# sunnyHelen/JPerceiver

Measured on AMD Instinct MI355X. Metric: train images/sec (full train step, synthetic 3-frame batches), higher is better.
Workload: dtype f32

## Files before the change

### jperceiver_amd/csrc/conv_pack.hip

```cpp
#include "conv_pack.h"
#include "igemm_p9.h"
#include "igemm_p9s.h"
#include "scale.h"
#include <algorithm>

namespace {

struct JpPackJob {
    const float* w;
    float* wp;
    long total, begin;
    int mode, p[6];
};
static_assert(sizeof(JpPackJob) == 64, "JpPackJob layout");
__host__ __device__ inline int jp_cdiv_d(int a, int b) { return (a + b - 1) / b; }

__device__ __forceinline__ float pack_slot_sum(const float* wc, int pl) {
    const int a = pl >> 3, b = (pl >> 2) & 1, r = (pl >> 1) & 1, sx = pl & 1;
    const int y0 = a ? (r ? 2 : 0) : (r ? 1 : 0), y1 = a ? (r ? 2 : 1) : (r ? 2 : 0);
    const int x0 = b ? (sx ? 2 : 0) : (sx ? 1 : 0), x1 = b ? (sx ? 2 : 1) : (sx ? 2 : 0);
    float v = 0.f;
    for (int dy = y0; dy <= y1; ++dy)
        for (int dx = x0; dx <= x1; ++dx) v += wc[dy * 3 + dx];
    return v;
// ... 165 lines not shown
        }
        default: {
            const int Cout = p[0], Cin = p[1], c_off = p[2];
            const int t = (int)(i % 9), co = (int)((i / 9) % Cout), c = (int)(i / (9 * (long)Cout));
            return w[((size_t)co * Cin + c_off + c) * 9 + 8 - t];
        }
    }
}

__device__ __forceinline__ int pack_hdr(int mode) { return (mode == PACK_SPLIT || mode == PACK_SPLITUPD || mode == PACK_SPLIT7) ? JP_PACK_HDR : 0; }
__device__ __forceinline__ float pack_scale_of(const JpPackJob& j) {
    if (!JP_PACK_HDR) return 1.f;
    if (j.mode == PACK_SPLIT || j.mode == PACK_SPLITUPD || j.mode == PACK_SPLIT7) return j.wp[0];
    if (j.mode == PACK_SPLITSEG) return *(j.wp - j.p[5]);
    return 1.f;
}
constexpr int PSL = 32;
__device__ __forceinline__ float* pack_scale_hdr(const JpPackJob& j, long* n) {
    const bool seg = j.mode == PACK_SPLITSEG && j.p[2] == 0;
    const bool upd = j.mode == PACK_SPLITUPD;
    const bool s7 = j.mode == PACK_SPLIT7;
    if (!JP_PACK_HDR || !(j.mode == PACK_SPLIT || seg || upd || s7)) return nullptr;
    *n = (long)j.p[0] * j.p[1] * ((seg || upd) ? 9 : (s7 ? 49 : j.p[4]));
    return seg ? j.wp - j.p[5] : j.wp;
}
__device__ __forceinline__ void pack_scale_zero(const JpPackJob& j) {
    long n;
    float* hdr = pack_scale_hdr(j, &n);
    if (hdr && threadIdx.x == 0) reinterpret_cast<unsigned*>(hdr)[2] = 0u;
}
__device__ __forceinline__ void pack_scale_reduce(const JpPackJob& j, int slice) {
    long n;
    float* hdr = pack_scale_hdr(j, &n);
    if (!hdr) return;
    const long per = (n + PSL - 1) / PSL, beg = slice * per, end = min(n, beg + per);
    unsigned m = 0;
    for (long i = beg + threadIdx.x; i < end; i += 256) m = max(m, jp_amag(__float_as_uint(j.w[i])));
#pragma unroll
    for (int o = 32; o > 0; o >>= 1) m = max(m, (unsigned)__shfl_xor((int)m, o, 64));
    if ((threadIdx.x & 63) == 0 && m) atomicMax(reinterpret_cast<unsigned*>(hdr) + 2, m);
}
__device__ __forceinline__ void pack_scale_finish(const JpPackJob& j) {
    long n;
    float* hdr = pack_scale_hdr(j, &n);
    if (!hdr || threadIdx.x) return;
    const int k = jp_scale_exp(hdr[2] * ((j.mode == PACK_SPLITSEG || j.mode == PACK_SPLITUPD) ? 4.f : 1.f));
    hdr[0] = jp_exp2i(k);
    hdr[1] = jp_exp2i(-k);
    hdr[2] = hdr[3] = 0.f;
}
__global__ __launch_bounds__(64) void pack_scale_zero_one_kernel(JpPackJob job) { pack_scale_zero(job); }
__global__ __launch_bounds__(256) void pack_scale_reduce_one_kernel(JpPackJob job) { pack_scale_reduce(job, blockIdx.x); }
__global__ __launch_bounds__(64) void pack_scale_finish_one_kernel(JpPackJob job) { pack_scale_finish(job); }
__global__ __launch_bounds__(64) void pack_scale_zero_kernel(const JpPackJob* __restrict__ jobs, int njobs) {
    const int q = blockIdx.x * 64 + threadIdx.x;
    if (q < njobs) { long n; float* hdr = pack_scale_hdr(jobs[q], &n); if (hdr) reinterpret_cast<unsigned*>(hdr)[2] = 0u; }
}
__global__ __launch_bounds__(256) void pack_scale_reduce_kernel(const JpPackJob* __restrict__ jobs, int njobs) {
    pack_scale_reduce(jobs[blockIdx.y], blockIdx.x);
}
__global__ __launch_bounds__(64) void pack_scale_finish_kernel(const JpPackJob* __restrict__ jobs, int njobs) {
    const int q = blockIdx.x * 64 + threadIdx.x;
    if (q < njobs) {
        long n;
        float* hdr = pack_scale_hdr(jobs[q], &n);
        if (hdr) {
            const int k = jp_scale_exp(hdr[2] * ((jobs[q].mode == PACK_SPLITSEG || jobs[q].mode == PACK_SPLITUPD) ? 4.f : 1.f));
            hdr[0] = jp_exp2i(k);
            hdr[1] = jp_exp2i(-k);
            hdr[2] = hdr[3] = 0.f;
        }
    }
}

__global__ __launch_bounds__(256) void pack_one_kernel(JpPackJob job) {
    const int hdr = pack_hdr(job.mode);
    const float sc = pack_scale_of(job);
    for (long i = (long)blockIdx.x * 256 + threadIdx.x; i < job.total - hdr; i += (long)gridDim.x * 256)
        job.wp[hdr + i] = pack_elem(job.mode, job.w, i, job.p, sc);
}

__global__ __launch_bounds__(256) void pack_replay_kernel(const JpPackJob* __restrict__ jobs, int njobs, long total) {
    const long groups = (total + 3) >> 2;
    for (long g4 = (long)blockIdx.x * 256 + threadIdx.x; g4 < groups; g4 += (long)gridDim.x * 256) {
        const long g = g4 << 2;
        int lo = 0, hi = njobs - 1;
        while (lo < hi) {
            const int mid = (lo + hi + 1) >> 1;
            if (jobs[mid].begin <= g) lo = mid; else hi = mid - 1;
        }
        const JpPackJob& j = jobs[lo];
        const long i = g - j.begin;
        if (i >= j.total) continue;
        if (j.mode == PACK_SPLIT || j.mode == PACK_SPLITSEG) continue;
        if (j.mode == PACK_FRAG && i + 4 <= j.total) {
            const int* p = j.p;
            const int Cout = p[0], Cin = p[1], for_dgrad = p[2], BMT = p[3], KHW = p[4];
            const int rows = for_dgrad ? Cin : Cout, red = for_dgrad ? Cout : Cin;
            const long per_tile = ((long)((red + 31) / 32) * KHW * 4 + P9_QAHEAD + 1) * 8 * BMT;
            const int mt = (int)(i / per_tile);
            long t = (i - (long)mt * per_tile) >> 2;
            const int m = mt * BMT + (int)(t % BMT);
            t /= BMT;
            const int par = (int)(t & 1); t >>= 1;
            const long step = t * 4;
            const int s0 = (int)(step & 15);
            const long tc = step >> 4;
            const int tap = (int)(tc % KHW), c0 = (int)(tc / KHW) * 32 + 2 * s0 + par;
            float4 v = make_float4(0.f, 0.f, 0.f, 0.f);
            if (m < rows) {
                const size_t cs = for_dgrad ? (size_t)Cin * KHW : (size_t)KHW;
                const float* wb = j.w + (for_dgrad ? (size_t)m * KHW : (size_t)m * Cin * KHW) + tap;
                if (c0 < red) v.x = wb[(size_t)c0 * cs];
                if (c0 + 2 < red) v.y = wb[(size_t)(c0 + 2) * cs];
                if (c0 + 4 < red) v.z = wb[(size_t)(c0 + 4) * cs];
                if (c0 + 6 < red) v.w = wb[(size_t)(c0 + 6) * cs];
            }
            *reinterpret_cast<float4*>(j.wp + i) = v;
        } else {
            const int hdr = pack_hdr(j.mode);
            const float sc = hdr ? pack_scale_of(j) : 1.f;
#pragma unroll
            for (int k = 0; k < 4; ++k)
                if (i + k >= hdr && i + k < j.total) j.wp[i + k] = pack_elem(j.mode, j.w, i + k - hdr, j.p, sc);
        }
    }
}

__device__ __forceinline__ int split_job_items(const JpPackJob& j) {
    const int* p = j.p;
    if (j.mode == PACK_SPLIT) {
        const int rows = p[2] ? p[1] : p[0], red = p[2] ? p[0] : p[1];
        return jp_cdiv_d(rows, p[3]) * (red / (16 * p[5])) * (p[3] / 64);
    }
    if (j.mode == PACK_SPLITSEG) return (p[0] / 128) * ((p[3] + 15) / 16) * 2;
    return 0;
}
__global__ __launch_bounds__(256) void pack_split_replay_kernel(const JpPackJob* __restrict__ jobs, int njobs) {
    __shared__ float tile[64 * 16 * 9 + 64];
    constexpr int MAXJ = 2048;
    __shared__ int pre[MAXJ + 1];
    const int t = threadIdx.x;
    for (int q = t; q < njobs && q < MAXJ; q += 256) pre[q + 1] = split_job_items(jobs[q]);
    if (t == 0) pre[0] = 0;
    __syncthreads();
    if (t == 0)
        for (int q = 1; q <= njobs && q <= MAXJ; ++q) pre[q] += pre[q - 1];
    __syncthreads();
    const int nj = min(njobs, MAXJ), total_items = pre[nj];
    for (int item = blockIdx.x; item < total_items; item += gridDim.x) {
        __syncthreads();
        int lo = 0, hi = nj - 1;
        while (lo < hi) {
            const int mid = (lo + hi + 1) >> 1;
            if (pre[mid] <= item) lo = mid; else hi = mid - 1;
        }
        const int jj = lo, loc = item - pre[lo];
        const JpPackJob& j = jobs[jj];
        const int* p = j.p;
        unsigned* out = reinterpret_cast<unsigned*>(j.wp) + pack_hdr(j.mode);
        if (j.mode == PACK_SPLIT) {
            const float wsc = JP_PACK_HDR ? j.wp[0] : 1.f;
            const int Cout = p[0], Cin = p[1], for_dgrad = p[2], BMT = p[3], KHW = p[4], KGS = p[5];
            const int rows = for_dgrad ? Cin : Cout, red = for_dgrad ? Cout : Cin;
            const int CS = 16 * KGS, nst = red / CS, rch = BMT / 64;
            const int rc = loc % rch, stage = (loc / rch) % nst, mt = loc / (rch * nst);
            const int m0 = mt * BMT + rc * 64, c0 = stage * CS;
            const int RUN = CS * KHW;
            if (!for_dgrad) {
                for (int e = t; e < 64 * RUN; e += 256) {
                    const int r = e / RUN, o = e - r * RUN;
                    tile[e] = (m0 + r < rows) ? j.w[((size_t)(m0 + r) * Cin + c0) * KHW + o] : 0.f;
                }
            } else {
                const int RUNd = 64 * KHW;
                for (int e = t; e < CS * RUNd; e += 256) {
                    const int c = e / RUNd, o = e - c * RUNd;
                    tile[e] = (m0 + o / KHW < rows) ? j.w[((size_t)(c0 + c) * Cin + m0) * KHW + o] : 0.f;
                }
            }
            __syncthreads();
            const long nsteps = (long)nst * KHW * KGS;
            const long per_tile = (nsteps + P9S_AHEAD) * (JP_NS * 8) * BMT;
            const int trip = KHW * KGS * 2 * 64;
            for (int e = t; e < trip; e += 256) {
                const int r = e & 63, kh = (e >> 6) & 1, u = e >> 7;
                const int tap = u / KGS, kg = u - tap * KGS;
                jp_u32x4 w0, w1, w2;
#pragma unroll
                for (int k = 0; k < 4; ++k) {
                    const int c = kg * 16 + kh * 8 + 2 * k;
                    const float a = for_dgrad ? tile[(c * 64 + r) * KHW + tap] : tile[(r * CS + c) * KHW + tap];
                    const float b = for_dgrad ? tile[((c + 1) * 64 + r) * KHW + tap] : tile[(r * CS + c + 1) * KHW + tap];
                    unsigned sq[3];
                    jp_split_ns(a, b, wsc, sq);
                    w0[k] = sq[0]; w1[k] = sq[1]; w2[k] = sq[2];
                }
                const long U = (long)stage * KHW * KGS + u;
                unsigned* q = out + (long)mt * per_tile + ((U * JP_NS) * 2 + kh) * (long)BMT * 4 + (long)(rc * 64 + r) * 4;
                *reinterpret_cast<jp_u32x4*>(q) = w0;
                *reinterpret_cast<jp_u32x4*>(q + 2L * BMT * 4) = w1;
                if (JP_NS == 3) *reinterpret_cast<jp_u32x4*>(q + 4L * BMT * 4) = w2;
            }
        } else {
            const int Cout = p[0], Cin = p[1], c_off = p[2], C = p[3], up = p[4];
            const int T = up ? 4 : 9, MT = Cout / 128, nst = (C + 15) / 16;
            const int rc = loc & 1, stage = (loc >> 1) % nst, mt = (loc >> 1) / nst;
            const int m0 = mt * 128 + rc * 64, c0 = stage * 16;
            for (int e = t; e < 64 * 144; e += 256) {
                const int r = e / 144, o = e - r * 144, c = o / 9;
                tile[e] = (c0 + c < C && m0 + r < Cout) ? j.w[((size_t)(m0 + r) * Cin + c_off + c0) * 9 + o] : 0.f;
            }
            __syncthreads();
            const long tl = (long)nst * T * (JP_NS * 1024);
            const int ncls = up ? 4 : 1, trip = ncls * T * 2 * 64;
            const float wsc = pack_scale_of(j);
            for (int e = t; e < trip; e += 256) {
                const int r = e & 63, kh = (e >> 6) & 1, ct = e >> 7, tap = ct % T, cls = ct / T;
                jp_u32x4 w0, w1, w2;
#pragma unroll
                for (int k = 0; k < 4; ++k) {
                    const int c = kh * 8 + 2 * k;
                    const float* wa = tile + (r * 16 + c) * 9;
                    const float a = up ? pack_slot_sum(wa, cls * 4 + tap) : wa[tap];
                    const float b = up ? pack_slot_sum(wa + 9, cls * 4 + tap) : wa[9 + tap];
                    unsigned sq[3];
                    jp_split_ns(a, b, wsc, sq);
                    w0[k] = sq[0]; w1[k] = sq[1]; w2[k] = sq[2];
                }
                const long U = (long)stage * T + tap;
                unsigned* q = out + (long)(cls * MT + mt) * tl + ((U * JP_NS) * 2 + kh) * 512L + (long)(rc * 64 + r) * 4;
                *reinterpret_cast<jp_u32x4*>(q) = w0;
                *reinterpret_cast<jp_u32x4*>(q + 1024) = w1;
                if (JP_NS == 3) *reinterpret_cast<jp_u32x4*>(q + 2048) = w2;
            }
        }
    }
}

thread_local JpPackJob* g_pack_rec = nullptr;
thread_local int g_pack_rec_n = 0, g_pack_rec_cap = 0;

}

void do_pack(int mode, const float* w, float* wp, long total, int p0, int p1, int p2, int p3, int p4, int p5, hipStream_t st) {
    JpPackJob j{w, wp, total, 0, mode, {p0, p1, p2, p3, p4, p5}};
    if (g_pack_rec) {
        if (g_pack_rec_n < g_pack_rec_cap) g_pack_rec[g_pack_rec_n] = j;
        ++g_pack_rec_n;
    }
    if (JP_PACK_HDR && (mode == PACK_SPLIT || mode == PACK_SPLITUPD || mode == PACK_SPLIT7 || (mode == PACK_SPLITSEG && p2 == 0))) {
        hipLaunchKernelGGL(pack_scale_zero_one_kernel, dim3(1), dim3(64), 0, st, j);
        hipLaunchKernelGGL(pack_scale_reduce_one_kernel, dim3(PSL), dim3(256), 0, st, j);
        hipLaunchKernelGGL(pack_scale_finish_one_kernel, dim3(1), dim3(64), 0, st, j);
    }
    hipLaunchKernelGGL(pack_one_kernel, dim3((int)std::min<long>((total + 255) / 256, 4096)), dim3(256), 0, st, j);
}

void pack_weights(const float* w, float* wp, int Cout, int Cin, int KHW, int Cp, int for_dgrad, hipStream_t st) {
    do_pack(PACK_TAP, w, wp, (long)KHW * (for_dgrad ? Cin : Cout) * Cp, Cout, Cin, KHW, Cp, for_dgrad, 0, st);
}

extern "C" int jp_pack_job_bytes(void) { return (int)sizeof(JpPackJob); }

extern "C" int jp_pack_record_begin(void* host_jobs, int max_jobs) {
    JP_CHECK_ARG(host_jobs && max_jobs > 0 && !g_pack_rec, "pack_record_begin: bad args or a recording is already open");
    g_pack_rec = (JpPackJob*)host_jobs;
    g_pack_rec_n = 0;
    g_pack_rec_cap = max_jobs;
    return JP_OK;
}

extern "C" int jp_pack_record_end(void) {
    g_pack_rec = nullptr;
    return g_pack_rec_n;
}

extern "C" int jp_pack_mode_is_split(int mode) { return (mode == PACK_SPLIT || mode == PACK_SPLITSEG) ? 1 : 0; }
extern "C" int jp_pack_replay(const void* jobs, int njobs, long total_elems, long generic_elems, void* stream) {
    JP_CHECK_ARG(jobs && njobs > 0 && total_elems > 0, "pack_replay: bad args");
    const long gen = (generic_elems > 0 && generic_elems < total_elems) ? generic_elems : total_elems;
    if (JP_PACK_HDR)
    {
        hipLaunchKernelGGL(pack_scale_zero_kernel, dim3((njobs + 63) / 64), dim3(64), 0, (hipStream_t)stream, (const JpPackJob*)jobs, njobs);
        hipLaunchKernelGGL(pack_scale_reduce_kernel, dim3(PSL, njobs), dim3(256), 0, (hipStream_t)stream, (const JpPackJob*)jobs, njobs);
        hipLaunchKernelGGL(pack_scale_finish_kernel, dim3((njobs + 63) / 64), dim3(64), 0, (hipStream_t)stream, (const JpPackJob*)jobs, njobs);
    }
    hipLaunchKernelGGL(pack_replay_kernel, dim3((int)std::min<long>((gen + 4095) / 4096, 16384)), dim3(256), 0,
                       (hipStream_t)stream, (const JpPackJob*)jobs, njobs, gen);
    for (int off = 0; off < njobs; off += 2048)
        hipLaunchKernelGGL(pack_split_replay_kernel, dim3(4096), dim3(256), 0, (hipStream_t)stream, (const JpPackJob*)jobs + off,
                           std::min(2048, njobs - off));
    JP_LAUNCH_CHECK();
}
```

### jperceiver_amd/csrc/pointwise.hip

```cpp
#include "jp_common.h"
#include "bilinear.h"
#include <algorithm>

namespace {

constexpr int TPB = 256;
inline int blocks_for(long n) { return (int)std::min<long>((n + TPB - 1) / TPB, 1 << 20); }

constexpr int MP_TW = 64, MP_TH = 8;

__global__ __launch_bounds__(TPB) void maxpool_fwd_kernel(const float* __restrict__ x, float* __restrict__ y,
                                                          uint8_t* __restrict__ idx, int H, int W, int OH, int OW,
                                                          int k, int s, int p) {
    extern __shared__ float tile[];
    const size_t nc = blockIdx.z;
    const float* xp = x + nc * H * W;
    const int ox0 = blockIdx.x * MP_TW, oy0 = blockIdx.y * MP_TH;
    const int pw = (MP_TW - 1) * s + k, ph = (MP_TH - 1) * s + k;
    const int ix0 = ox0 * s - p, iy0 = oy0 * s - p;
    for (int i = threadIdx.x; i < pw * ph; i += TPB) {
        const int ly = i / pw, lx = i - ly * pw;
        const int iy = iy0 + ly, ix = ix0 + lx;
        tile[i] = ((unsigned)iy < (unsigned)H && (unsigned)ix < (unsigned)W) ? xp[iy * W + ix] : -INFINITY;
    }
// ... 628 lines not shown
            mx = fmaxf(mx, jp_fmag(o));
            fs += o;
            if (++run == 32) { s += fs; fs = 0.f; run = 0; }
        }
    }
    jp_block_amax_commit(mx, amax);
    s += fs;
    s = jp_block_sum_d(s, sm);
    if (threadIdx.x == 0) {
        if (part) part[(size_t)c * gridDim.y + blockIdx.y] = (float)s;
        else atomicAdd(&dbias[c], (float)s);
    }
}
__global__ void bias_fold_kernel(const float* __restrict__ part, float* __restrict__ dbias, int C, int S) {
    const int c = blockIdx.x * blockDim.x + threadIdx.x;
    if (c >= C) return;
    float s = 0.f;
    for (int i = 0; i < S; ++i) s += part[(size_t)c * S + i];
    dbias[c] += s;
}

__global__ __launch_bounds__(TPB) void mul_bcast_c_kernel(const float* __restrict__ a, const float* __restrict__ s,
                                                          float* __restrict__ out, long total, int C, int HW) {
    for (long i = (long)blockIdx.x * TPB + threadIdx.x; i < total; i += (long)gridDim.x * TPB) {
        const int p = (int)(i % HW);
        const long n = i / ((long)C * HW);
        out[i] = a[i] * s[n * HW + p];
    }
}
__global__ __launch_bounds__(TPB) void mul_bcast_c_bwd_s_kernel(const float* __restrict__ dout,
                                                                const float* __restrict__ a, float* __restrict__ ds,
                                                                long total, int C, int HW) {
    for (long i = (long)blockIdx.x * TPB + threadIdx.x; i < total; i += (long)gridDim.x * TPB) {
        const int p = (int)(i % HW);
        const long n = i / HW;
        float g = 0.f;
        for (int c = 0; c < C; ++c) g += dout[(n * C + c) * HW + p] * a[(n * C + c) * HW + p];
        ds[i] = g;
    }
}

__global__ __launch_bounds__(TPB) void bilinear_fwd_kernel(const float* __restrict__ x, float* __restrict__ y,
                                                           long total, int H, int W, int OH, int OW, float sy,
                                                           float sx) {
    for (long o = (long)blockIdx.x * TPB + threadIdx.x; o < total; o += (long)gridDim.x * TPB) {
        const int ox = (int)(o % OW);
        const long t = o / OW;
        const int oy = (int)(t % OH);
        const long nc = t / OH;
        y[o] = bil_sample(x + nc * H * W, oy, ox, H, W, sy, sx);
    }
}

__global__ __launch_bounds__(TPB) void bilinear_bwd_kernel(const float* __restrict__ dy, float* __restrict__ dx,
                                                           long total, int H, int W, int OH, int OW, float sy,
                                                           float sx, int accumulate) {
    for (long i = (long)blockIdx.x * TPB + threadIdx.x; i < total; i += (long)gridDim.x * TPB) {
        const int ix = (int)(i % W);
        const long t = i / W;
        const int iy = (int)(t % H);
        const long nc = t / H;
        const float* dp = dy + nc * OH * OW;
        int oy_lo = max(0, (int)floorf(((float)iy - 0.5f) / sy - 0.5f) - 1);
        int oy_hi = min(OH - 1, (int)ceilf(((float)iy + 1.5f) / sy - 0.5f) + 1);
        int ox_lo = max(0, (int)floorf(((float)ix - 0.5f) / sx - 0.5f) - 1);
        int ox_hi = min(OW - 1, (int)ceilf(((float)ix + 1.5f) / sx - 0.5f) + 1);
        if (iy == 0) oy_lo = 0;
        if (ix == 0) ox_lo = 0;
        if (iy == H - 1) oy_hi = OH - 1;
        if (ix == W - 1) ox_hi = OW - 1;
        float g = 0.f;
        for (int oy = oy_lo; oy <= oy_hi; ++oy) {
            int y0, y1;
            float wy;
            bil_src(oy, sy, H, y0, y1, wy);
            float cy = 0.f;
            if (y0 == iy) cy += 1.f - wy;
            if (y1 == iy) cy += wy;
            if (cy == 0.f) continue;
            for (int ox = ox_lo; ox <= ox_hi; ++ox) {
                int x0, x1;
                float wx;
                bil_src(ox, sx, W, x0, x1, wx);
                float cx = 0.f;
                if (x0 == ix) cx += 1.f - wx;
                if (x1 == ix) cx += wx;
                if (cx != 0.f) g += cy * cx * dp[oy * OW + ox];
            }
        }
        dx[i] = accumulate ? dx[i] + g : g;
    }
}

__global__ __launch_bounds__(TPB) void area_down_kernel(const float* __restrict__ x, float* __restrict__ y,
                                                        long total, int H, int W, int OH, int OW, int f) {
    const float inv = 1.f / (float)(f * f);
    for (long o = (long)blockIdx.x * TPB + threadIdx.x; o < total; o += (long)gridDim.x * TPB) {
        const int ox = (int)(o % OW);
        const long t = o / OW;
        const int oy = (int)(t % OH);
        const long nc = t / OH;
        const float* xp = x + (nc * H + (long)oy * f) * W + (long)ox * f;
        float s = 0.f;
        for (int a = 0; a < f; ++a)
            for (int b = 0; b < f; ++b) s += xp[a * W + b];
        y[o] = s * inv;
    }
}

__global__ __launch_bounds__(TPB) void warp_perspective_kernel(const float* __restrict__ src,
                                                               const float* __restrict__ Hm, float* __restrict__ dst,
                                                               int h, int w, int OH, int OW) {
    const int b = blockIdx.y;
    const float* M = Hm + 9 * b;
    const float* sp = src + (size_t)b * h * w;
    for (int p = blockIdx.x * TPB + threadIdx.x; p < OH * OW; p += gridDim.x * TPB) {
        const int oy = p / OW, ox = p - oy * OW;
        const float gx = OW > 1 ? -1.f + 2.f * (float)ox / (float)(OW - 1) : -1.f;
        const float gy = OH > 1 ? -1.f + 2.f * (float)oy / (float)(OH - 1) : -1.f;
        const float X = M[0] * gx + M[1] * gy + M[2];
        const float Y = M[3] * gx + M[4] * gy + M[5];
        const float Z = M[6] * gx + M[7] * gy + M[8];
        const float sx = X / Z, sy = Y / Z;
        const float ix = ((sx + 1.f) * (float)w - 1.f) * 0.5f, iy = ((sy + 1.f) * (float)h - 1.f) * 0.5f;
        const float fx = floorf(ix), fy = floorf(iy);
        const int x0 = (int)fx, y0 = (int)fy;
        const float tx = ix - fx, ty = iy - fy;
        float v = 0.f;
        if (ix == ix && iy == iy && fx > -2.f && fy > -2.f && fx < (float)w + 1.f && fy < (float)h + 1.f) {
            const bool xa = x0 >= 0 && x0 < w, xb = x0 + 1 >= 0 && x0 + 1 < w;
            const bool ya = y0 >= 0 && y0 < h, yb = y0 + 1 >= 0 && y0 + 1 < h;
            if (ya && xa) v += sp[y0 * w + x0] * (1.f - tx) * (1.f - ty);
            if (ya && xb) v += sp[y0 * w + x0 + 1] * tx * (1.f - ty);
            if (yb && xa) v += sp[(y0 + 1) * w + x0] * (1.f - tx) * ty;
            if (yb && xb) v += sp[(y0 + 1) * w + x0 + 1] * tx * ty;
        }
        dst[(size_t)b * OH * OW + p] = v;
    }
}

__global__ __launch_bounds__(TPB) void softmax_c2_kernel(const float* __restrict__ x, float* __restrict__ y,
                                                         long total, int HW) {
    for (long i = (long)blockIdx.x * TPB + threadIdx.x; i < total; i += (long)gridDim.x * TPB) {
// ... 307 lines not shown
    int ch = std::max(1, 2048 / std::max(1, N * C));
    ch = std::min(ch, std::max(1, HW / 2048));
    int ck = (HW + ch - 1) / ch;
    ck = (ck + 3) & ~3;
    *chunk = ck;
    *CH = (HW + ck - 1) / ck;
}
extern "C" long jp_act_bwd_bias_ws_floats(int N, int C, int HW) {
    int CH, chunk;
    act_bias_chunks(N, C, HW, &CH, &chunk);
    return (long)C * N * CH;
}
extern "C" int jp_act_bwd_bias(const float* dy, const float* y, float* dx, float* dbias, int N, int C, int HW, int act,
                               float* amax_dx, float* bias_ws, void* stream) {
    JP_CHECK_ARG(dy && y && dx && dbias && N > 0 && C > 0 && HW > 0 && C <= 65535, "act_bwd_bias: bad args");
    JP_ST;
    int CH, chunk;
    act_bias_chunks(N, C, HW, &CH, &chunk);
    JP_CHECK_ARG((long)N * CH <= 65535, "act_bwd_bias: too many chunks");
    hipLaunchKernelGGL(act_bwd_bias_kernel, dim3(C, N * CH), dim3(TPB), 0, st, dy, y, dx, dbias, C, HW, CH, chunk, act,
                       reinterpret_cast<unsigned*>(amax_dx), bias_ws);
    if (bias_ws) hipLaunchKernelGGL(bias_fold_kernel, dim3(jp_cdiv(C, 64)), dim3(64), 0, st, bias_ws, dbias, C, N * CH);
    JP_LAUNCH_CHECK();
}

extern "C" int jp_mul_bcast_c(const float* a, const float* s, float* out, int N, int C, int HW, void* stream) {
    JP_CHECK_ARG(a && s && out && N > 0, "mul_bcast_c: bad args");
    JP_ST;
    const long total = (long)N * C * HW;
    hipLaunchKernelGGL(mul_bcast_c_kernel, dim3(blocks_for(total)), dim3(TPB), 0, st, a, s, out, total, C, HW);
    JP_LAUNCH_CHECK();
}

extern "C" int jp_mul_bcast_c_bwd_s(const float* dout, const float* a, float* ds, int N, int C, int HW,
                                    void* stream) {
    JP_CHECK_ARG(dout && a && ds && N > 0, "mul_bcast_c_bwd_s: bad args");
    JP_ST;
    const long total = (long)N * HW;
    hipLaunchKernelGGL(mul_bcast_c_bwd_s_kernel, dim3(blocks_for(total)), dim3(TPB), 0, st, dout, a, ds, total, C, HW);
    JP_LAUNCH_CHECK();
}

extern "C" int jp_bilinear_fwd(const float* x, float* y, int NC, int H, int W, int OH, int OW, void* stream) {
    JP_CHECK_ARG(x && y && NC > 0 && OH > 0 && OW > 0, "bilinear_fwd: bad args");
    JP_ST;
    const long total = (long)NC * OH * OW;
    hipLaunchKernelGGL(bilinear_fwd_kernel, dim3(blocks_for(total)), dim3(TPB), 0, st, x, y, total, H, W, OH, OW,
                       (float)H / (float)OH, (float)W / (float)OW);
    JP_LAUNCH_CHECK();
}

extern "C" int jp_bilinear_bwd(const float* dy, float* dx, int NC, int H, int W, int OH, int OW, int accumulate,
                               void* stream) {
    JP_CHECK_ARG(dy && dx && NC > 0, "bilinear_bwd: bad args");
    JP_ST;
    const long total = (long)NC * H * W;
    hipLaunchKernelGGL(bilinear_bwd_kernel, dim3(blocks_for(total)), dim3(TPB), 0, st, dy, dx, total, H, W, OH, OW,
                       (float)H / (float)OH, (float)W / (float)OW, accumulate);
    JP_LAUNCH_CHECK();
}

extern "C" int jp_area_downsample(const float* x, float* y, int NC, int H, int W, int f, void* stream) {
    JP_CHECK_ARG(x && y && NC > 0 && f >= 1 && H % f == 0 && W % f == 0, "area_downsample: bad args");
    JP_ST;
    const long total = (long)NC * (H / f) * (W / f);
    hipLaunchKernelGGL(area_down_kernel, dim3(blocks_for(total)), dim3(TPB), 0, st, x, y, total, H, W, H / f, W / f, f);
    JP_LAUNCH_CHECK();
}

extern "C" int jp_warp_perspective(const float* src, const float* Hm, float* dst, int B, int h, int w, int OH, int OW,
                                   void* stream) {
    JP_CHECK_ARG(src && Hm && dst && B > 0, "warp_perspective: bad args");
    JP_ST;
    hipLaunchKernelGGL(warp_perspective_kernel, dim3(std::min(jp_cdiv((long)OH * OW, TPB), 4096), B), dim3(TPB), 0, st,
                       src, Hm, dst, h, w, OH, OW);
    JP_LAUNCH_CHECK();
}

extern "C" int jp_softmax_c2(const float* x, float* y, int N, int HW, void* stream) {
    JP_CHECK_ARG(x && y && N > 0 && HW > 0, "softmax_c2: bad args");
    JP_ST;
    const long total = (long)N * HW;
    hipLaunchKernelGGL(softmax_c2_kernel, dim3(blocks_for(total)), dim3(TPB), 0, st, x, y, total, HW);
    JP_LAUNCH_CHECK();
}

extern "C" int jp_disp_to_depth(const float* disp, float* depth, long n, float min_depth, float max_depth,
                                void* stream) {
    JP_CHECK_ARG(disp && depth && n > 0, "disp_to_depth: bad args");
    JP_ST;
    hipLaunchKernelGGL(disp_to_depth_kernel, dim3(blocks_for(n)), dim3(TPB), 0, st, disp, depth, n, 1.f / max_depth,
                       1.f / min_depth);
    JP_LAUNCH_CHECK();
}

extern "C" int jp_fill_convex_poly(const int* pts, int npts, uint8_t* mask, int H, int W, void* stream) {
    JP_CHECK_ARG(pts && mask && npts >= 1 && npts <= POLY_MAX && H > 0 && W > 0, "fill_convex_poly: bad args");
    JP_ST;
    JP_HIP(hipMemsetAsync(mask, 0, (size_t)H * W, st));
    hipLaunchKernelGGL(fill_convex_poly_kernel, dim3(8), dim3(TPB), 0, st, pts, npts, mask, H, W);
    JP_LAUNCH_CHECK();
}

extern "C" int jp_scale_label_assemble(const float* zwarp, const float* laywarp, const uint8_t* polymask, float* out,
                                       int B, int H, int W, int mode, void* stream) {
    JP_CHECK_ARG(zwarp && out && B > 0 && (mode == 0 || polymask), "scale_label_assemble: bad args");
    JP_ST;
    const long total = (long)B * H * W;
    hipLaunchKernelGGL(scale_label_kernel, dim3(blocks_for(total)), dim3(TPB), 0, st, zwarp, laywarp, polymask, out,
                       total, (long)H * W, mode);
    JP_LAUNCH_CHECK();
// ... 2 lines not shown
```

Measured before the change: 128.5.

## Restructure weight-pack replay and separable bilinear backward with shared-memory staging

Weight packing now builds its job prefix with a parallel wave scan and runs the scale-max reduction as a flat work list with vectorized loads. Several more pack modes (tap, up-dgrad, split-update) are staged through shared-memory tiles with coalesced run fills, and launch sizes are tied to the CU count. Bilinear backward becomes separable: each block reduces the output rows into a shared horizontal buffer once, then each thread gathers along x. This cuts repeated per-pixel window scans and redundant global reads. The cost is more code and a risk of mishandling edge cases.

```diff
diff --git a/jperceiver_amd/csrc/conv_pack.hip b/jperceiver_amd/csrc/conv_pack.hip
--- a/jperceiver_amd/csrc/conv_pack.hip
+++ b/jperceiver_amd/csrc/conv_pack.hip
@@ -241,12 +241,84 @@
 __global__ __launch_bounds__(64) void pack_scale_zero_one_kernel(JpPackJob job) { pack_scale_zero(job); }
 __global__ __launch_bounds__(256) void pack_scale_reduce_one_kernel(JpPackJob job) { pack_scale_reduce(job, blockIdx.x); }
 __global__ __launch_bounds__(64) void pack_scale_finish_one_kernel(JpPackJob job) { pack_scale_finish(job); }
-__global__ __launch_bounds__(64) void pack_scale_zero_kernel(const JpPackJob* __restrict__ jobs, int njobs) {
-    const int q = blockIdx.x * 64 + threadIdx.x;
-    if (q < njobs) { long n; float* hdr = pack_scale_hdr(jobs[q], &n); if (hdr) reinterpret_cast<unsigned*>(hdr)[2] = 0u; }
+constexpr int PACK_MAXJ = 2048;
+template <class F>
+__device__ __forceinline__ int pack_item_prefix(const JpPackJob* __restrict__ jobs, int nj, int* pre, F items_of) {
+    constexpr int PER = PACK_MAXJ / 256;
+    __shared__ int wave_sum[4];
+    const int t = threadIdx.x, lane = t & 63, wv = t >> 6;
+    int cnt[PER], sum = 0;
+#pragma unroll
+    for (int k = 0; k < PER; ++k) {
+        const int q = t * PER + k;
+        cnt[k] = q < nj ? items_of(jobs[q]) : 0;
+        sum += cnt[k];
+    }
+    int inc = sum;
+#pragma unroll
+    for (int o = 1; o < 64; o <<= 1) {
+        const int v = __shfl_up(inc, o, 64);
+        if (lane >= o) inc += v;
+    }
+    if (lane == 63) wave_sum[wv] = inc;
+    __syncthreads();
+    int run = inc - sum;
+    for (int k = 0; k < wv; ++k) run += wave_sum[k];
+    if (t == 0) pre[0] = 0;
+#pragma unroll
+    for (int k = 0; k < PER; ++k) {
+        const int q = t * PER + k;
+        run += cnt[k];
+        if (q < nj) pre[q + 1] = run;
+    }
+    __syncthreads();
+    return pre[nj];
+}
+__device__ __forceinline__ int pack_item_job(const int* pre, int nj, int item) {
+    int lo = 0, hi = nj - 1;
+    while (lo < hi) {
+        const int mid = (lo + hi + 1) >> 1;
+        if (pre[mid] <= item) lo = mid; else hi = mid - 1;
+    }
+    return lo;
+}
+
+constexpr int PACK_RED_ITEM = 16384;
+__device__ __forceinline__ int scale_job_items(const JpPackJob& j) {
+    long n;
+    return pack_scale_hdr(j, &n) ? (int)((n + PACK_RED_ITEM - 1) / PACK_RED_ITEM) : 0;
 }
 __global__ __launch_bounds__(256) void pack_scale_reduce_kernel(const JpPackJob* __restrict__ jobs, int njobs) {
-    pack_scale_reduce(jobs[blockIdx.y], blockIdx.x);
+    __shared__ int pre[PACK_MAXJ + 1];
+    __shared__ unsigned wave_max[4];
+    const int t = threadIdx.x;
+    const int total_items = pack_item_prefix(jobs, njobs, pre, scale_job_items);
+    for (int item = blockIdx.x; item < total_items; item += gridDim.x) {
+        const int jj = pack_item_job(pre, njobs, item);
+        const JpPackJob& j = jobs[jj];
+        long n;
+        float* hdr = pack_scale_hdr(j, &n);
+        const long beg = (long)(item - pre[jj]) * PACK_RED_ITEM, end = min(n, beg + PACK_RED_ITEM);
+        const float* w = j.w;
+        const long a0 = min(end, beg + (long)((4 - (int)((reinterpret_cast<size_t>(w + beg) >> 2) & 3)) & 3));
+        const long nv = (end - a0) >> 2;
+        unsigned m = 0;
+        for (long i = beg + t; i < a0; i += 256) m = max(m, jp_amag(__float_as_uint(w[i])));
+        for (long i = t; i < nv; i += 256) {
+            const jp_u32x4 v = *reinterpret_cast<const jp_u32x4*>(w + a0 + 4 * i);
+            m = max(max(m, jp_amag(v[0])), max(max(jp_amag(v[1]), jp_amag(v[2])), jp_amag(v[3])));
+        }
+        for (long i = a0 + 4 * nv + t; i < end; i += 256) m = max(m, jp_amag(__float_as_uint(w[i])));
+#pragma unroll
+        for (int o = 32; o > 0; o >>= 1) m = max(m, (unsigned)__shfl_xor((int)m, o, 64));
+        if ((t & 63) == 0) wave_max[t >> 6] = m;
+        __syncthreads();
+        if (t == 0) {
+            m = max(max(wave_max[0], wave_max[1]), max(wave_max[2], wave_max[3]));
+            if (m) atomicMax(reinterpret_cast<unsigned*>(hdr) + 2, m);
+        }
+        __syncthreads();
+    }
 }
 __global__ __launch_bounds__(64) void pack_scale_finish_kernel(const JpPackJob* __restrict__ jobs, int njobs) {
     const int q = blockIdx.x * 64 + threadIdx.x;
@@ -269,53 +341,61 @@
         job.wp[hdr + i] = pack_elem(job.mode, job.w, i, job.p, sc);
 }
 
+__host__ __device__ inline bool pack_mode_staged(int mode) {
+    return mode == PACK_SPLIT || mode == PACK_SPLITSEG || mode == PACK_TAP || mode == PACK_UP_DGRAD || mode == PACK_SPLITUPD;
+}
+__device__ __forceinline__ void pack_replay_group(const JpPackJob& j, long i) {
+    if (i >= j.total) return;
+    if (pack_mode_staged(j.mode)) return;
+    if (j.mode == PACK_FRAG && i + 4 <= j.total) {
+        const int* p = j.p;
+        const int Cout = p[0], Cin = p[1], for_dgrad = p[2], BMT = p[3], KHW = p[4];
+        const int rows = for_dgrad ? Cin : Cout, red = for_dgrad ? Cout : Cin;
+        const long per_tile = ((long)((red + 31) / 32) * KHW * 4 + P9_QAHEAD + 1) * 8 * BMT;
+        const int mt = (int)(i / per_tile);
+        long t = (i - (long)mt * per_tile) >> 2;
+        const int m = mt * BMT + (int)(t % BMT);
+        t /= BMT;
+        const int par = (int)(t & 1); t >>= 1;
+        const long step = t * 4;
+        const int s0 = (int)(step & 15);
+        const long tc = step >> 4;
+        const int tap = (int)(tc % KHW), c0 = (int)(tc / KHW) * 32 + 2 * s0 + par;
+        float4 v = make_float4(0.f, 0.f, 0.f, 0.f);
+        if (m < rows) {
+            const size_t cs = for_dgrad ? (size_t)Cin * KHW : (size_t)KHW;
+            const float* wb = j.w + (for_dgrad ? (size_t)m * KHW : (size_t)m * Cin * KHW) + tap;
+            if (c0 < red) v.x = wb[(size_t)c0 * cs];
+            if (c0 + 2 < red) v.y = wb[(size_t)(c0 + 2) * cs];
+            if (c0 + 4 < red) v.z = wb[(size_t)(c0 + 4) * cs];
+            if (c0 + 6 < red) v.w = wb[(size_t)(c0 + 6) * cs];
+        }
+        *reinterpret_cast<float4*>(j.wp + i) = v;
+    } else {
+        const int hdr = pack_hdr(j.mode);
+        const float sc = hdr ? pack_scale_of(j) : 1.f;
+#pragma unroll
+        for (int k = 0; k < 4; ++k)
+            if (i + k >= hdr && i + k < j.total) j.wp[i + k] = pack_elem(j.mode, j.w, i + k - hdr, j.p, sc);
+    }
+}
+
 __global__ __launch_bounds__(256) void pack_replay_kernel(const JpPackJob* __restrict__ jobs, int njobs, long total) {
     const long groups = (total + 3) >> 2;
-    for (long g4 = (long)blockIdx.x * 256 + threadIdx.x; g4 < groups; g4 += (long)gridDim.x * 256) {
-        const long g = g4 << 2;
+    for (long cb = (long)blockIdx.x * 256; cb < groups; cb += (long)gridDim.x * 256) {
         int lo = 0, hi = njobs - 1;
         while (lo < hi) {
             const int mid = (lo + hi + 1) >> 1;
-            if (jobs[mid].begin <= g) lo = mid; else hi = mid - 1;
-        }
-        const JpPackJob& j = jobs[lo];
-        const long i = g - j.begin;
-        if (i >= j.total) continue;
-        if (j.mode == PACK_SPLIT || j.mode == PACK_SPLITSEG) continue;
-        if (j.mode == PACK_FRAG && i + 4 <= j.total) {
-            const int* p = j.p;
-            const int Cout = p[0], Cin = p[1], for_dgrad = p[2], BMT = p[3], KHW = p[4];
-            const int rows = for_dgrad ? Cin : Cout, red = for_dgrad ? Cout : Cin;
-            const long per_tile = ((long)((red + 31) / 32) * KHW * 4 + P9_QAHEAD + 1) * 8 * BMT;
-            const int mt = (int)(i / per_tile);
-            long t = (i - (long)mt * per_tile) >> 2;
-            const int m = mt * BMT + (int)(t % BMT);
-            t /= BMT;
-            const int par = (int)(t & 1); t >>= 1;
-            const long step = t * 4;
-            const int s0 = (int)(step & 15);
-            const long tc = step >> 4;
-            const int tap = (int)(tc % KHW), c0 = (int)(tc / KHW) * 32 + 2 * s0 + par;
-            float4 v = make_float4(0.f, 0.f, 0.f, 0.f);
-            if (m < rows) {
-                const size_t cs = for_dgrad ? (size_t)Cin * KHW : (size_t)KHW;
-                const float* wb = j.w + (for_dgrad ? (size_t)m * KHW : (size_t)m * Cin * KHW) + tap;
-                if (c0 < red) v.x = wb[(size_t)c0 * cs];
-                if (c0 + 2 < red) v.y = wb[(size_t)(c0 + 2) * cs];
-                if (c0 + 4 < red) v.z = wb[(size_t)(c0 + 4) * cs];
-                if (c0 + 6 < red) v.w = wb[(size_t)(c0 + 6) * cs];
-            }
-            *reinterpret_cast<float4*>(j.wp + i) = v;
-        } else {
-            const int hdr = pack_hdr(j.mode);
-            const float sc = hdr ? pack_scale_of(j) : 1.f;
-#pragma unroll
-            for (int k = 0; k < 4; ++k)
-                if (i + k >= hdr && i + k < j.total) j.wp[i + k] = pack_elem(j.mode, j.w, i + k - hdr, j.p, sc);
-        }
-    }
-}
-
+            if (jobs[mid].begin <= (cb << 2)) lo = mid; else hi = mid - 1;
+        }
+        const long g = (cb + threadIdx.x) << 2;
+        if (g >= total) continue;
+        while (lo + 1 < njobs && jobs[lo + 1].begin <= g) ++lo;
+        pack_replay_group(jobs[lo], g - jobs[lo].begin);
+    }
+}
+
+__device__ __forceinline__ int tap_item_rows(int KHW) { return min(64, 9216 / (64 * KHW)); }
 __device__ __forceinline__ int split_job_items(const JpPackJob& j) {
     const int* p = j.p;
     if (j.mode == PACK_SPLIT) {
@@ -323,28 +403,49 @@
         return jp_cdiv_d(rows, p[3]) * (red / (16 * p[5])) * (p[3] / 64);
     }
     if (j.mode == PACK_SPLITSEG) return (p[0] / 128) * ((p[3] + 15) / 16) * 2;
+    if (j.mode == PACK_TAP) {
+        const int rows = p[4] ? p[1] : p[0], R = tap_item_rows(p[2]);
+        return R ? jp_cdiv_d(rows, R) * jp_cdiv_d(p[3], 64) : (int)((j.total + 4095) / 4096);
+    }
+    if (j.mode == PACK_UP_DGRAD) return jp_cdiv_d(p[3], 16) * jp_cdiv_d(p[4], 64);
+    if (j.mode == PACK_SPLITUPD) return jp_cdiv_d(p[3], 128) * ((p[0] + 31) / 32 * 2) * 2;
     return 0;
 }
+__device__ __forceinline__ void pack_fill_runs(float* tile, int pitch, const float* __restrict__ src, long stride, int nruns, int run,
+                                               int valid, int nvalid) {
+    const int t = threadIdx.x;
+    if (((reinterpret_cast<size_t>(src) >> 2 | (size_t)stride | (size_t)run | (size_t)valid) & 3) == 0) {
+        const int q = run >> 2, dq = 256 / q, dr = 256 - dq * q;
+        int i = t / q, o = t - i * q;
+        const bool wide = (pitch & 3) == 0;
+        while (i < nruns) {
+            float4 v = make_float4(0.f, 0.f, 0.f, 0.f);
+            if (i < nvalid && 4 * o < valid) v = *reinterpret_cast<const float4*>(src + i * stride + 4 * o);
+            float* d = tile + i * pitch + 4 * o;
+            if (wide) *reinterpret_cast<float4*>(d) = v;
+            else { d[0] = v.x; d[1] = v.y; d[2] = v.z; d[3] = v.w; }
+            i += dq; o += dr;
+            if (o >= q) { o -= q; ++i; }
+        }
+    } else {
+        const int dq = 256 / run, dr = 256 - dq * run;
+        int i = t / run, o = t - i * run;
+        while (i < nruns) {
+            tile[i * pitch + o] = (i < nvalid && o < valid) ? src[i * stride + o] : 0.f;
+            i += dq; o += dr;
+            if (o >= run) { o -= run; ++i; }
+        }
+    }
+}
 __global__ __launch_bounds__(256) void pack_split_replay_kernel(const JpPackJob* __restrict__ jobs, int njobs) {
-    __shared__ float tile[64 * 16 * 9 + 64];
-    constexpr int MAXJ = 2048;
-    __shared__ int pre[MAXJ + 1];
+    __shared__ __attribute__((aligned(16))) float tile[64 * (16 * 9 + 1)];
+    __shared__ int pre[PACK_MAXJ + 1];
     const int t = threadIdx.x;
-    for (int q = t; q < njobs && q < MAXJ; q += 256) pre[q + 1] = split_job_items(jobs[q]);
-    if (t == 0) pre[0] = 0;
-    __syncthreads();
-    if (t == 0)
-        for (int q = 1; q <= njobs && q <= MAXJ; ++q) pre[q] += pre[q - 1];
-    __syncthreads();
-    const int nj = min(njobs, MAXJ), total_items = pre[nj];
+    const int nj = min(njobs, PACK_MAXJ);
+    const int total_items = pack_item_prefix(jobs, nj, pre, split_job_items);
     for (int item = blockIdx.x; item < total_items; item += gridDim.x) {
         __syncthreads();
-        int lo = 0, hi = nj - 1;
-        while (lo < hi) {
-            const int mid = (lo + hi + 1) >> 1;
-            if (pre[mid] <= item) lo = mid; else hi = mid - 1;
-        }
-        const int jj = lo, loc = item - pre[lo];
+        const int jj = pack_item_job(pre, nj, item), loc = item - pre[jj];
         const JpPackJob& j = jobs[jj];
         const int* p = j.p;
         unsigned* out = reinterpret_cast<unsigned*>(j.wp) + pack_hdr(j.mode);
@@ -355,34 +456,24 @@
             const int CS = 16 * KGS, nst = red / CS, rch = BMT / 64;
             const int rc = loc % rch, stage = (loc / rch) % nst, mt = loc / (rch * nst);
             const int m0 = mt * BMT + rc * 64, c0 = stage * CS;
-            const int RUN = CS * KHW;
-            if (!for_dgrad) {
-                for (int e = t; e < 64 * RUN; e += 256) {
-                    const int r = e / RUN, o = e - r * RUN;
-                    tile[e] = (m0 + r < rows) ? j.w[((size_t)(m0 + r) * Cin + c0) * KHW + o] : 0.f;
-                }
-            } else {
-                const int RUNd = 64 * KHW;
-                for (int e = t; e < CS * RUNd; e += 256) {
-                    const int c = e / RUNd, o = e - c * RUNd;
-                    tile[e] = (m0 + o / KHW < rows) ? j.w[((size_t)(c0 + c) * Cin + m0) * KHW + o] : 0.f;
-                }
-            }
+            const int RUN = CS * KHW, PITCH = RUN | 1;
+            const int RUNd = 64 * KHW, live = min(64, rows - m0);
+            if (!for_dgrad) pack_fill_runs(tile, PITCH, j.w + ((size_t)m0 * Cin + c0) * KHW, (long)Cin * KHW, 64, RUN, RUN, live);
+            else pack_fill_runs(tile, RUNd, j.w + ((size_t)c0 * Cin + m0) * KHW, (long)Cin * KHW, CS, RUNd, live * KHW, CS);
             __syncthreads();
             const long nsteps = (long)nst * KHW * KGS;
             const long per_tile = (nsteps + P9S_AHEAD) * (JP_NS * 8) * BMT;
             const int trip = KHW * KGS * 2 * 64;
+            const int cstr = for_dgrad ? RUNd : KHW, rstr = for_dgrad ? KHW : PITCH;
             for (int e = t; e < trip; e += 256) {
                 const int r = e & 63, kh = (e >> 6) & 1, u = e >> 7;
                 const int tap = u / KGS, kg = u - tap * KGS;
+                const float* ta = tile + r * rstr + (kg * 16 + kh * 8) * cstr + tap;
                 jp_u32x4 w0, w1, w2;
 #pragma unroll
                 for (int k = 0; k < 4; ++k) {
-                    const int c = kg * 16 + kh * 8 + 2 * k;
-                    const float a = for_dgrad ? tile[(c * 64 + r) * KHW + tap] : tile[(r * CS + c) * KHW + tap];
-                    const float b = for_dgrad ? tile[((c + 1) * 64 + r) * KHW + tap] : tile[(r * CS + c + 1) * KHW + tap];
                     unsigned sq[3];
-                    jp_split_ns(a, b, wsc, sq);
+                    jp_split_ns(ta[2 * k * cstr], ta[(2 * k + 1) * cstr], wsc, sq);
                     w0[k] = sq[0]; w1[k] = sq[1]; w2[k] = sq[2];
                 }
                 const long U = (long)stage * KHW * KGS + u;
@@ -391,15 +482,79 @@
                 *reinterpret_cast<jp_u32x4*>(q + 2L * BMT * 4) = w1;
                 if (JP_NS == 3) *reinterpret_cast<jp_u32x4*>(q + 4L * BMT * 4) = w2;
             }
+        } else if (j.mode == PACK_TAP) {
+            const int Cout = p[0], Cin = p[1], KHW = p[2], Cp = p[3], for_dgrad = p[4];
+            const int rows = for_dgrad ? Cin : Cout, red = for_dgrad ? Cout : Cin;
+            const int R = tap_item_rows(KHW);
+            if (R == 0) {
+                for (long i = (long)loc * 4096 + t; i < min(j.total, (long)(loc + 1) * 4096); i += 256) j.wp[i] = pack_elem(PACK_TAP, j.w, i, p);
+                continue;
+            }
+            const int nck = jp_cdiv_d(Cp, 64), ck = loc % nck, r0 = (loc / nck) * R, cc0 = ck * 64;
+            const int wc = min(64, Cp - cc0), live_c = max(0, min(wc, red - cc0)), live_r = min(R, rows - r0);
+            const int pitch = ((for_dgrad ? R : 64) * KHW) | 1;
+            if (!for_dgrad) pack_fill_runs(tile, pitch, j.w + ((size_t)r0 * Cin + cc0) * KHW, (long)Cin * KHW, R, wc * KHW, live_c * KHW, live_r);
+            else pack_fill_runs(tile, pitch, j.w + ((size_t)cc0 * Cin + r0) * KHW, (long)Cin * KHW, wc, R * KHW, live_r * KHW, live_c);
+            __syncthreads();
+            const int cstr = for_dgrad ? pitch : KHW, rstr = for_dgrad ? KHW : pitch;
+            const int lines = KHW * live_r;
+            if (256 % wc == 0) {
+                const int c = t % wc, dl = 256 / wc, dtap = dl / live_r, dr = dl - dtap * live_r;
+                int y = t / wc, tap = y / live_r, r = y - tap * live_r;
+                for (; y < lines; y += dl) {
+                    j.wp[((size_t)tap * rows + r0 + r) * Cp + cc0 + c] = tile[c * cstr + r * rstr + tap];
+                    tap += dtap; r += dr;
+                    if (r >= live_r) { r -= live_r; ++tap; }
+                }
+            } else {
+                for (int e = t; e < lines * wc; e += 256) {
+                    const int y = e / wc, c = e - y * wc, tap = y / live_r, r = y - tap * live_r;
+                    j.wp[((size_t)tap * rows + r0 + r) * Cp + cc0 + c] = tile[c * cstr + r * rstr + tap];
+                }
+            }
+        } else if (j.mode == PACK_UP_DGRAD) {
+            const int Cout = p[0], Cin = p[1], c_off = p[2], Cx = p[3], Cp = p[4];
+            const int nck = jp_cdiv_d(Cp, 64), co0 = (loc % nck) * 64, c0 = (loc / nck) * 16;
+            const int wc = min(64, Cp - co0), live_c = min(16, Cx - c0);
+            pack_fill_runs(tile, 145, j.w + ((size_t)co0 * Cin + c_off + c0) * 9, (long)Cin * 9, 64, 144, live_c * 9, max(0, min(64, Cout - co0)));
+            __syncthreads();
+            for (int e = t; e < 16 * live_c * wc; e += 256) {
+                const int y = e / wc, co = e - y * wc, pl = y / live_c, c = y - pl * live_c;
+                j.wp[((size_t)pl * Cx + c0 + c) * Cp + co0 + co] = pack_slot_sum(tile + co * 145 + c * 9, pl);
+            }
+        } else if (j.mode == PACK_SPLITUPD) {
+            const int Cout = p[0], Cin = p[1], c_off = p[2], Cx = p[3];
+            const int nst = (Cout + 31) / 32 * 2;
+            const int rc = loc & 1, stage = (loc >> 1) % nst, mt = (loc >> 1) / nst;
+            const int r0 = mt * 128 + rc * 64, co0 = stage * 16;
+            pack_fill_runs(tile, 576, j.w + ((size_t)co0 * Cin + c_off + r0) * 9, (long)Cin * 9, 16, 576, max(0, min(64, Cx - r0)) * 9,
+                           max(0, min(16, Cout - co0)));
+            __syncthreads();
+            const long per_tile = ((long)nst * 16 + P9S_AHEAD) * (JP_NS * 1024);
+            const float wsc = pack_scale_of(j);
+            for (int e = t; e < 16 * 2 * 64; e += 256) {
+                const int r = e & 63, kh = (e >> 6) & 1, q = e >> 7;
+                jp_u32x4 w0, w1, w2;
+#pragma unroll
+                for (int k = 0; k < 4; ++k) {
+                    const float* wa = tile + (kh * 8 + 2 * k) * 576 + r * 9;
+                    unsigned sq[3];
+                    jp_split_ns(pack_slot_sum(wa, q), pack_slot_sum(wa + 576, q), wsc, sq);
+                    w0[k] = sq[0]; w1[k] = sq[1]; w2[k] = sq[2];
+                }
+                const long U = (long)stage * 16 + q;
+                unsigned* d = out + (long)mt * per_tile + ((U * JP_NS) * 2 + kh) * 512L + (long)(rc * 64 + r) * 4;
+                *reinterpret_cast<jp_u32x4*>(d) = w0;
+                *reinterpret_cast<jp_u32x4*>(d + 1024) = w1;
+                if (JP_NS == 3) *reinterpret_cast<jp_u32x4*>(d + 2048) = w2;
+            }
         } else {
             const int Cout = p[0], Cin = p[1], c_off = p[2], C = p[3], up = p[4];
             const int T = up ? 4 : 9, MT = Cout / 128, nst = (C + 15) / 16;
             const int rc = loc & 1, stage = (loc >> 1) % nst, mt = (loc >> 1) / nst;
             const int m0 = mt * 128 + rc * 64, c0 = stage * 16;
-            for (int e = t; e < 64 * 144; e += 256) {
-                const int r = e / 144, o = e - r * 144, c = o / 9;
-                tile[e] = (c0 + c < C && m0 + r < Cout) ? j.w[((size_t)(m0 + r) * Cin + c_off + c0) * 9 + o] : 0.f;
-            }
+            pack_fill_runs(tile, 145, j.w + ((size_t)m0 * Cin + c_off + c0) * 9, (long)Cin * 9, 64, 144, min(16, C - c0) * 9,
+                           min(64, Cout - m0));
             __syncthreads();
             const long tl = (long)nst * T * (JP_NS * 1024);
             const int ncls = up ? 4 : 1, trip = ncls * T * 2 * 64;
@@ -410,7 +565,7 @@
 #pragma unroll
                 for (int k = 0; k < 4; ++k) {
                     const int c = kh * 8 + 2 * k;
-                    const float* wa = tile + (r * 16 + c) * 9;
+                    const float* wa = tile + r * 145 + c * 9;
                     const float a = up ? pack_slot_sum(wa, cls * 4 + tap) : wa[tap];
                     const float b = up ? pack_slot_sum(wa + 9, cls * 4 + tap) : wa[9 + tap];
                     unsigned sq[3];
@@ -465,20 +620,25 @@
     return g_pack_rec_n;
 }
 
-extern "C" int jp_pack_mode_is_split(int mode) { return (mode == PACK_SPLIT || mode == PACK_SPLITSEG) ? 1 : 0; }
+extern "C" int jp_pack_mode_is_split(int mode) { return pack_mode_staged(mode) ? 1 : 0; }
 extern "C" int jp_pack_replay(const void* jobs, int njobs, long total_elems, long generic_elems, void* stream) {
     JP_CHECK_ARG(jobs && njobs > 0 && total_elems > 0, "pack_replay: bad args");
     const long gen = (generic_elems > 0 && generic_elems < total_elems) ? generic_elems : total_elems;
+    static const int cus = [] {
+        int dev = 0, v = 256;
+        if (hipGetDevice(&dev) == hipSuccess) (void)hipDeviceGetAttribute(&v, hipDeviceAttributeMultiprocessorCount, dev);
+        return v > 0 ? v : 256;
+    }();
+    const JpPackJob* jt = (const JpPackJob*)jobs;
+    hipStream_t st = (hipStream_t)stream;
     if (JP_PACK_HDR)
     {
-        hipLaunchKernelGGL(pack_scale_zero_kernel, dim3((njobs + 63) / 64), dim3(64), 0, (hipStream_t)stream, (const JpPackJob*)jobs, njobs);
-        hipLaunchKernelGGL(pack_scale_reduce_kernel, dim3(PSL, njobs), dim3(256), 0, (hipStream_t)stream, (const JpPackJob*)jobs, njobs);
-        hipLaunchKernelGGL(pack_scale_finish_kernel, dim3((njobs + 63) / 64), dim3(64), 0, (hipStream_t)stream, (const JpPackJob*)jobs, njobs);
-    }
-    hipLaunchKernelGGL(pack_replay_kernel, dim3((int)std::min<long>((gen + 4095) / 4096, 16384)), dim3(256), 0,
-                       (hipStream_t)stream, (const JpPackJob*)jobs, njobs, gen);
-    for (int off = 0; off < njobs; off += 2048)
-        hipLaunchKernelGGL(pack_split_replay_kernel, dim3(4096), dim3(256), 0, (hipStream_t)stream, (const JpPackJob*)jobs + off,
-                           std::min(2048, njobs - off));
+        for (int off = 0; off < njobs; off += PACK_MAXJ)
+            hipLaunchKernelGGL(pack_scale_reduce_kernel, dim3(cus * 8), dim3(256), 0, st, jt + off, std::min(PACK_MAXJ, njobs - off));
+        hipLaunchKernelGGL(pack_scale_finish_kernel, dim3((njobs + 63) / 64), dim3(64), 0, st, jt, njobs);
+    }
+    hipLaunchKernelGGL(pack_replay_kernel, dim3((int)std::min<long>((gen + 1023) / 1024, 16384)), dim3(256), 0, st, jt, njobs, gen);
+    for (int off = 0; off < njobs; off += PACK_MAXJ)
+        hipLaunchKernelGGL(pack_split_replay_kernel, dim3(cus * 3), dim3(256), 0, st, jt + off, std::min(PACK_MAXJ, njobs - off));
     JP_LAUNCH_CHECK();
 }
diff --git a/jperceiver_amd/csrc/pointwise.hip b/jperceiver_amd/csrc/pointwise.hip
--- a/jperceiver_amd/csrc/pointwise.hip
+++ b/jperceiver_amd/csrc/pointwise.hip
@@ -704,43 +704,77 @@
     }
 }
 
-__global__ __launch_bounds__(TPB) void bilinear_bwd_kernel(const float* __restrict__ dy, float* __restrict__ dx,
-                                                           long total, int H, int W, int OH, int OW, float sy,
-                                                           float sx, int accumulate) {
-    for (long i = (long)blockIdx.x * TPB + threadIdx.x; i < total; i += (long)gridDim.x * TPB) {
-        const int ix = (int)(i % W);
-        const long t = i / W;
-        const int iy = (int)(t % H);
-        const long nc = t / H;
+__device__ __forceinline__ void bil_adj_window(int i, float s, int in, int on, int& lo, int& hi) {
+    lo = max(0, (int)floorf(((float)i - 0.5f) / s - 0.5f) - 1);
+    hi = min(on - 1, (int)ceilf(((float)i + 1.5f) / s - 0.5f) + 1);
+    if (i == 0) lo = 0;
+    if (i == in - 1) hi = on - 1;
+}
+__device__ __forceinline__ float bil_adj_weight(int o, float s, int in, int i) {
+    int i0, i1;
+    float w1;
+    bil_src(o, s, in, i0, i1, w1);
+    return (i0 == i ? 1.f - w1 : 0.f) + (i1 == i ? w1 : 0.f);
+}
+constexpr int BB_TX = 256, BB_K = 5, BB_HB = BB_TX * BB_K;
+constexpr int BB_M = 4;
+__global__ __launch_bounds__(BB_TX) void bilinear_bwd_kernel(const float* __restrict__ dy, float* __restrict__ dx,
+                                                             long nblk, int xch, int tx, int H, int W, int OH, int OW, float sy,
+                                                             float sx, int accumulate) {
+    __shared__ float h[BB_HB];
+    const int t = threadIdx.x;
+    for (long b = blockIdx.x; b < nblk; b += gridDim.x) {
+        const int xc = (int)(b % xch);
+        const long r = b / xch;
+        const int iy = (int)(r % H);
+        const long nc = r / H;
         const float* dp = dy + nc * OH * OW;
-        int oy_lo = max(0, (int)floorf(((float)iy - 0.5f) / sy - 0.5f) - 1);
-        int oy_hi = min(OH - 1, (int)ceilf(((float)iy + 1.5f) / sy - 0.5f) + 1);
-        int ox_lo = max(0, (int)floorf(((float)ix - 0.5f) / sx - 0.5f) - 1);
-        int ox_hi = min(OW - 1, (int)ceilf(((float)ix + 1.5f) / sx - 0.5f) + 1);
-        if (iy == 0) oy_lo = 0;
-        if (ix == 0) ox_lo = 0;
-        if (iy == H - 1) oy_hi = OH - 1;
-        if (ix == W - 1) ox_hi = OW - 1;
-        float g = 0.f;
-        for (int oy = oy_lo; oy <= oy_hi; ++oy) {
-            int y0, y1;
-            float wy;
-            bil_src(oy, sy, H, y0, y1, wy);
-            float cy = 0.f;
-            if (y0 == iy) cy += 1.f - wy;
-            if (y1 == iy) cy += wy;
-            if (cy == 0.f) continue;
-            for (int ox = ox_lo; ox <= ox_hi; ++ox) {
-                int x0, x1;
-                float wx;
-                bil_src(ox, sx, W, x0, x1, wx);
-                float cx = 0.f;
-                if (x0 == ix) cx += 1.f - wx;
-                if (x1 == ix) cx += wx;
-                if (cx != 0.f) g += cy * cx * dp[oy * OW + ox];
-            }
-        }
-        dx[i] = accumulate ? dx[i] + g : g;
+        const int ix0 = xc * tx, ixl = min(W, ix0 + tx) - 1;
+        int oy_lo, oy_hi, wlo, whi, tmp, my_lo[BB_M], my_hi[BB_M];
+        bil_adj_window(iy, sy, H, OH, oy_lo, oy_hi);
+        bil_adj_window(ix0, sx, W, OW, wlo, tmp);
+        bil_adj_window(ixl, sx, W, OW, tmp, whi);
+        float g[BB_M];
+#pragma unroll
+        for (int m = 0; m < BB_M; ++m) {
+            g[m] = 0.f;
+            my_lo[m] = 0;
+            my_hi[m] = -1;
+            if (ix0 + t + m * BB_TX <= ixl) bil_adj_window(ix0 + t + m * BB_TX, sx, W, OW, my_lo[m], my_hi[m]);
+        }
+        for (int base = wlo; base <= whi; base += BB_HB) {
+            const int n = min(BB_HB, whi - base + 1);
+            float a[BB_K];
+#pragma unroll
+            for (int k = 0; k < BB_K; ++k) a[k] = 0.f;
+#pragma unroll 4
+            for (int oy = oy_lo; oy <= oy_hi; ++oy) {
+                const float cy = bil_adj_weight(oy, sy, H, iy);
+                const float* rp = dp + (long)oy * OW + base;
+#pragma unroll
+                for (int k = 0; k < BB_K; ++k)
+                    if (t + k * BB_TX < n) {
+                        const float v = rp[t + k * BB_TX];
+                        a[k] += cy != 0.f ? cy * v : 0.f;
+                    }
+            }
+#pragma unroll
+            for (int k = 0; k < BB_K; ++k)
+                if (t + k * BB_TX < n) h[t + k * BB_TX] = a[k];
+            __syncthreads();
+#pragma unroll
+            for (int m = 0; m < BB_M; ++m) {
+                const int e = min(my_hi[m], base + n - 1);
+                for (int ox = max(my_lo[m], base); ox <= e; ++ox) g[m] += bil_adj_weight(ox, sx, W, ix0 + t + m * BB_TX) * h[ox - base];
+            }
+            __syncthreads();
+        }
+#pragma unroll
+        for (int m = 0; m < BB_M; ++m)
+            if (ix0 + t + m * BB_TX <= ixl) {
+                float* o = dx + (nc * H + iy) * W + ix0 + t + m * BB_TX;
+                *o = accumulate ? *o + g[m] : g[m];
+            }
     }
 }
 
@@ -1154,11 +1188,14 @@
 
 extern "C" int jp_bilinear_bwd(const float* dy, float* dx, int NC, int H, int W, int OH, int OW, int accumulate,
                                void* stream) {
-    JP_CHECK_ARG(dy && dx && NC > 0, "bilinear_bwd: bad args");
-    JP_ST;
-    const long total = (long)NC * H * W;
-    hipLaunchKernelGGL(bilinear_bwd_kernel, dim3(blocks_for(total)), dim3(TPB), 0, st, dy, dx, total, H, W, OH, OW,
-                       (float)H / (float)OH, (float)W / (float)OW, accumulate);
+    JP_CHECK_ARG(dy && dx && NC > 0 && H > 0 && W > 0 && OH > 0 && OW > 0, "bilinear_bwd: bad args");
+    JP_ST;
+    const float sy = (float)H / (float)OH, sx = (float)W / (float)OW;
+    const int tx = BB_TX * std::max(1, std::min(BB_M, (int)(((BB_HB - 4) * sx - 2.f) / BB_TX)));
+    const int xch = (W + tx - 1) / tx;
+    const long nblk = (long)NC * H * xch;
+    hipLaunchKernelGGL(bilinear_bwd_kernel, dim3((int)std::min<long>(nblk, 1 << 20)), dim3(BB_TX), 0, st, dy, dx, nblk, xch, tx, H, W,
+                       OH, OW, sy, sx, accumulate);
     JP_LAUNCH_CHECK();
 }
 
```

Measured after the change: 129.9 (median of 6 runs). +1.1%, better.
